# kureta/ddsp-pytorch

Measured on AMD Instinct MI355X. Metric: audio samples/sec/GPU + %HBM-roofline, 16kHz/100-harmonic/batch512, higher is better.
Workload: dtype f32

## Files before the change

ddsp-pytorch_amd/csrc/ddsp_noise_wave.hip:

```cpp
#include <hip/hip_runtime.h>
#include <stdint.h>

#include <atomic>

#include "ddsp_hip.h"
#include "ddsp_internal.h"
#include "ddsp_noise_common.h"

using namespace ddsp_noise;

namespace {

typedef float v4f __attribute__((ext_vector_type(4)));

struct Tile { v4f v[5]; };
struct Lines { v4f v[8]; };
struct Pass { float v[16]; };
struct Spectra { v4f e[2], o[2], h64; float z32; };

constexpr int R = kWaveHop;
constexpr int F = kWaveBands;
constexpr int FG = kWaveGroupFrames;
static_assert(R == 128 && F == 65 && FG == 16 && 2 * (F - 1) == R, "the kernel's register and LDS layouts are written for these");
constexpr int KS = 132;
constexpr int XS = 140;
constexpr int kLdsFloats = FG * KS + FG * XS;

#ifndef DDSP_NOISE_ABL
#define DDSP_NOISE_ABL 0
#endif

#ifdef DDSP_NOISE_STAMPS
#define DDSP_STAMP(i) do { asm volatile("s_waitcnt lgkmcnt(0)" ::: "memory"); const unsigned long long now_ = __builtin_amdgcn_s_memtime(); \
                           stamp_sum[i] += now_ - stamp_last; stamp_last = now_; } while (0)
#else
#define DDSP_STAMP(i) do { } while (0)
#endif

template <bool ACC>
__global__ void __launch_bounds__(64, 2) noise_wave_kernel(NoiseParams p, long ngroups)
{
    extern __shared__ __attribute__((aligned(16))) float smem[];
    float *kern = smem;
    float *xs = smem + FG * KS;
    float *Hs = kern, *ys = xs;
    const int lane = threadIdx.x;
#ifdef DDSP_NOISE_STAMPS
    unsigned long long stamp_sum[8] = {0, 0, 0, 0, 0, 0, 0, 0}, stamp_last = __builtin_amdgcn_s_memtime();
    unsigned long long *stamp_out = reinterpret_cast<unsigned long long *>(const_cast<float *>(p.u)) + 8 * blockIdx.x;
    p.u = nullptr;
#endif

    const int mi0 = lane & 15, mq0 = lane >> 4;
    float *ctab = xs;
    ctab[lane] = cospif((float)lane * (1.0f / 64.0f));
    ctab[lane + 64] = cospif((float)(lane + 64) * (1.0f / 64.0f));
    DDSP_WAVE_ORDER();
    Split Be[2], Bo[2];
#pragma unroll
    for (int t = 0; t < 2; ++t) {
        const int n = 16 * t + mi0;
#pragma unroll
        for (int j = 0; j < 8; ++j) {
            const int k = 8 * mq0 + j;
            split3((k == 0 ? 0.5f : 1.0f) * ctab[(2 * k * n) & 127], Be[t], j);
            split3(ctab[((2 * k + 1) * n) & 127], Bo[t], j);
        }
    }
    float w1[2], w2[2];
#pragma unroll
    for (int t = 0; t < 2; ++t) {
        const int n = 16 * t + mi0;
        w1[t] = __fmaf_rn(0.5f, ctab[n], 0.5f) * (1.0f / 64.0f);
        w2[t] = __fmaf_rn(0.5f, ctab[64 - n], 0.5f) * (1.0f / 64.0f);
    }
    DDSP_WAVE_ORDER();
    const uint64_t base_off = p.offset + (p.offset_dev ? *p.offset_dev : 0ull);

    auto load_tile = [&](long g) {
        const v4f *src = reinterpret_cast<const v4f *>(p.Hm + g * FG * F);
        Tile h;
#pragma unroll
        for (int j = 0; j < 4; ++j) h.v[j] = src[lane + 64 * j];
        h.v[4] = src[256 + (lane & 3)];
        return h;
    };

    auto opaque_lane = [&]() { int ln = lane; asm volatile("" : "+v"(ln)); return ln; };

    auto products = [&](const Tile h) {
        const int ln = opaque_lane(), mi = ln & 15, mq = ln >> 4;
#pragma unroll
        for (int j = 0; j < 4; ++j) *reinterpret_cast<v4f *>(Hs + 4 * (ln + 64 * j)) = h.v[j];
        if (ln < 4) *reinterpret_cast<v4f *>(Hs + 4 * (ln + 256)) = h.v[4];
        DDSP_WAVE_ORDER();
        const float *hrow = Hs + mi * F + 16 * mq;
        float hv[16];
#pragma unroll
        for (int j = 0; j < 16; ++j) hv[j] = hrow[j];
        const float h64 = Hs[mi * F + 64];
        Spectra sp;
#pragma unroll
        for (int r = 0; r < 4; ++r) sp.h64[r] = 0.5f * Hs[(4 * mq + r) * F + 64];
        DDSP_WAVE_ORDER();
        Split Ae, Ao;
#pragma unroll
        for (int j = 0; j < 8; ++j) { split3(hv[2 * j], Ae, j); split3(hv[2 * j + 1], Ao, j); }
        v4f (&accE)[2] = sp.e, (&accO)[2] = sp.o;
        accE[0] = accE[1] = accO[0] = accO[1] = (v4f){0, 0, 0, 0};
        constexpr int PA[6] = {2, 1, 0, 1, 0, 0}, PB[6] = {0, 1, 2, 0, 1, 0};
#pragma unroll
        for (int i = 0; i < (DDSP_NOISE_ABL == 3 ? 1 : 6); ++i) {
            accE[0] = __builtin_amdgcn_mfma_f32_16x16x32_bf16(Ae.p[PA[i]], Be[0].p[PB[i]], accE[0], 0, 0, 0);
            accE[1] = __builtin_amdgcn_mfma_f32_16x16x32_bf16(Ae.p[PA[i]], Be[1].p[PB[i]], accE[1], 0, 0, 0);
            accO[0] = __builtin_amdgcn_mfma_f32_16x16x32_bf16(Ao.p[PA[i]], Bo[0].p[PB[i]], accO[0], 0, 0, 0);
            accO[1] = __builtin_amdgcn_mfma_f32_16x16x32_bf16(Ao.p[PA[i]], Bo[1].p[PB[i]], accO[1], 0, 0, 0);
        }
        float t = (mq == 0 ? 0.5f : 1.0f) * hv[0];
#pragma unroll
        for (int j = 1; j < 8; ++j) t += (j & 1) ? -hv[2 * j] : hv[2 * j];
        t += __shfl_xor(t, 16);
        t += __shfl_xor(t, 32);
        sp.z32 = (t + 0.5f * h64) * (0.5f / 64.0f);
        return sp;
    };

    auto taps = [&](const Spectra sp) {
        const int ln = opaque_lane(), mi = ln & 15, mq = ln >> 4;
        const v4f (&accE)[2] = sp.e, (&accO)[2] = sp.o;
        const float z32 = sp.z32;
#pragma unroll
        for (int t = 0; t < 2; ++t) {
            const int n = 16 * t + mi;
#pragma unroll
            for (int r = 0; r < 4; ++r) {
                float *kr = kern + (4 * mq + r) * KS;
                const float ev = accE[t][r] + ((mi & 1) ? -sp.h64[r] : sp.h64[r]);
                const float v1 = (ev + accO[t][r]) * w1[t];
                const float v2 = (ev - accO[t][r]) * w2[t];
                kr[n] = v1;
                if (n != 0) { kr[128 - n] = v1; kr[64 - n] = v2; }
                kr[64 + n] = v2;
            }
        }
        if (mq == 0) { kern[mi * KS + 32] = z32; kern[mi * KS + 96] = z32; }
        DDSP_WAVE_ORDER();
    };

    auto draw = [&](long frame0) {
        const int ln = opaque_lane();
        for (int e = ln; e < FG * 8; e += 64) xs[(e >> 3) * XS + (e & 7)] = 0.0f;
        if (p.u) {
#pragma unroll
            for (int j = 0; j < 8; ++j) {
                const int qi = ln + 64 * j, fr = qi >> 5, q = qi & 31;
                float4 v = *reinterpret_cast<const float4 *>(p.u + (frame0 + fr) * R + 4 * q);
                v.x = v.x * 2.0f - 1.0f; v.y = v.y * 2.0f - 1.0f; v.z = v.z * 2.0f - 1.0f; v.w = v.w * 2.0f - 1.0f;
                *reinterpret_cast<float4 *>(xs + fr * XS + 8 + 4 * q) = v;
            }
        } else {
            const uint64_t c0 = base_off + (uint64_t)frame0 * 32u + (uint64_t)ln;
#pragma unroll
            for (int j = 0; j < 8; ++j) {
                const int qi = ln + 64 * j, fr = qi >> 5, q = qi & 31;
                const uint64_t ctr = c0 + 64u * j;
                uint32_t rr[4];
                if (DDSP_NOISE_ABL == 2) { rr[0] = (uint32_t)ctr; rr[1] = rr[0] * 3u; rr[2] = rr[0] ^ 77u; rr[3] = rr[0] + 5u; }
                else philox4x32_10((uint32_t)ctr, (uint32_t)(ctr >> 32), (uint32_t)p.seed, (uint32_t)(p.seed >> 32), rr);
                float4 v;
                v.x = philox_to_sample(rr[0]); v.y = philox_to_sample(rr[1]); v.z = philox_to_sample(rr[2]); v.w = philox_to_sample(rr[3]);
                *reinterpret_cast<float4 *>(xs + fr * XS + 8 + 4 * q) = v;
            }
        }
        DDSP_WAVE_ORDER();
    };

    auto conv_pass = [&](int pass) {
        const int ln = opaque_lane();
        const int l5 = ln & 31, seg = l5 >> 2;
        const int cf = ((seg >> 1) << 2) | (l5 & 3);
        const int cs = 2 * (ln >> 5) + ((0x96 >> seg) & 1);
        const float *krow = kern + cf * KS;
        const float *xrow = xs + cf * XS + 8;
        const int cA = pass ? 8 + cs : 15 - cs, cB = 15 - cA;
        const int tsw = cA + 1;
        const float *kq_a = krow, *kq_b = krow - 8 * tsw;
        const float *xq_a = xrow + 8 * cA - 8 - 128, *xq_b = xrow + 8 * cB - 8 + 8 * tsw - 128;
        float acc[8], first[8];
#pragma unroll
        for (int u = 0; u < 8; ++u) { acc[u] = 0.0f; first[u] = 0.0f; }
        float4 cur[6], nxt[6];
        auto fetch = [&](float4 (&d)[6], const float *kq, const float *xq, int t) {
            d[0] = *reinterpret_cast<const float4 *>(kq + 8 * t);
            d[1] = *reinterpret_cast<const float4 *>(kq + 8 * t + 4);
            d[2] = *reinterpret_cast<const float4 *>(xq + 8 * (16 - t));
            d[3] = *reinterpret_cast<const float4 *>(xq + 8 * (16 - t) + 4);
            d[4] = *reinterpret_cast<const float4 *>(xq + 8 * (16 - t) + 8);
            d[5] = *reinterpret_cast<const float4 *>(xq + 8 * (16 - t) + 12);
        };
        fetch(cur, kq_a, xq_a, 0);
#pragma unroll
        for (int t = 0; t < (DDSP_NOISE_ABL == 1 ? 1 : 17); ++t) {
            if (t < 16) {
                if (t + 1 < 9) fetch(nxt, kq_a, xq_a, t + 1);
                else { const bool b = t + 1 >= tsw; fetch(nxt, b ? kq_b : kq_a, b ? xq_b : xq_a, t + 1); }
            }
            if (t >= 9 && t == tsw) {
                asm volatile("" ::: "memory");
#pragma unroll
                for (int u = 0; u < 8; ++u) { first[u] = acc[u]; acc[u] = 0.0f; }
            }
            asm volatile("" ::"v"(cur[2].x));
            const float kv[8] = {cur[0].x, cur[0].y, cur[0].z, cur[0].w, cur[1].x, cur[1].y, cur[1].z, cur[1].w};
            const float xw[16] = {cur[2].x, cur[2].y, cur[2].z, cur[2].w, cur[3].x, cur[3].y, cur[3].z, cur[3].w,
                                  cur[4].x, cur[4].y, cur[4].z, cur[4].w, cur[5].x, cur[5].y, cur[5].z, cur[5].w};
#pragma unroll
            for (int v = 0; v < 8; ++v)
#pragma unroll
                for (int u = 0; u < 8; ++u) acc[u] = __fmaf_rn(kv[v], xw[8 + u - v], acc[u]);
#pragma unroll
            for (int e = 0; e < 6; ++e) cur[e] = nxt[e];
            __builtin_amdgcn_sched_barrier(0);
        }
        Pass out;
#pragma unroll
        for (int u = 0; u < 8; ++u) { out.v[u] = first[u]; out.v[8 + u] = acc[u]; }
        return out;
    };

    auto stage = [&](const Pass r0, const Pass r1) {
        const int ln = opaque_lane();
        const int l5 = ln & 31, seg = l5 >> 2;
        const int cf = ((seg >> 1) << 2) | (l5 & 3);
        const int cs = 2 * (ln >> 5) + ((0x96 >> seg) & 1);
        DDSP_WAVE_ORDER();
#pragma unroll
        for (int pass = 0; pass < 2; ++pass) {
            const float (&r)[16] = pass ? r1.v : r0.v;
            const int cA = pass ? 8 + cs : 15 - cs, cB = 15 - cA;
            float *ya = ys + cf * KS + 8 * cA, *yb = ys + cf * KS + 8 * cB;
            *reinterpret_cast<float4 *>(ya) = make_float4(r[0], r[1], r[2], r[3]);
            *reinterpret_cast<float4 *>(ya + 4) = make_float4(r[4], r[5], r[6], r[7]);
            *reinterpret_cast<float4 *>(yb) = make_float4(r[8], r[9], r[10], r[11]);
            *reinterpret_cast<float4 *>(yb + 4) = make_float4(r[12], r[13], r[14], r[15]);
        }
        DDSP_WAVE_ORDER();
    };

    auto read_y = [&](long frame0) {
        const v4f *src = reinterpret_cast<const v4f *>(p.y) + frame0 * (R / 4);
        Lines yv;
#pragma unroll
        for (int j = 0; j < 8; ++j) yv.v[j] = src[lane + 64 * j];
        return yv;
    };
    auto store_y = [&](long frame0, const Lines yv) {
        const int ln = opaque_lane();
        v4f *dst = reinterpret_cast<v4f *>(p.y) + frame0 * (R / 4);
#pragma unroll
        for (int j = 0; j < 8; ++j) {
            const int i4 = ln + 64 * j;
            v4f o = *reinterpret_cast<const v4f *>(ys + (i4 >> 5) * KS + 4 * (i4 & 31));
            if (ACC && DDSP_NOISE_ABL != 4) o += yv.v[j];
            if (DDSP_NOISE_ABL != 4 || o[0] == 123.0f) dst[i4] = o;
        }
        DDSP_WAVE_ORDER();
    };

    long g = blockIdx.x;
    if (g >= ngroups) return;
    Tile hreg = load_tile(g);
    Lines yv;
#pragma unroll
    for (int j = 0; j < 8; ++j) yv.v[j] = (v4f){0.0f, 0.0f, 0.0f, 0.0f};
    taps(products(hreg));
    draw(g * FG);
    DDSP_STAMP(0);
    for (;;) {
        {
            const unsigned slot = (unsigned)__builtin_amdgcn_s_getreg((4 << 0) | (0 << 6) | (3 << 11));
            const unsigned epoch = (unsigned)(__builtin_amdgcn_s_memrealtime() >> 12);
            if ((slot + epoch) & 1u) __builtin_amdgcn_s_setprio(1); else __builtin_amdgcn_s_setprio(0);
        }
        const long frame0 = g * FG;
        const long gn = g + gridDim.x;
        const Pass r0 = conv_pass(0);
        DDSP_STAMP(1);
        hreg = load_tile(gn < ngroups ? gn : g);
        if (ACC && DDSP_NOISE_ABL != 4) yv = read_y(frame0);
        const Pass r1 = conv_pass(1);
        DDSP_STAMP(2);
        stage(r0, r1);
        DDSP_STAMP(3);
        if (gn >= ngroups) break;
        const Spectra sp = products(hreg);
        DDSP_STAMP(4);
        store_y(frame0, yv);
        DDSP_STAMP(5);
        taps(sp);
        DDSP_STAMP(6);
        draw(gn * FG);
        DDSP_STAMP(7);
        g = gn;
    }
    store_y(g * FG, yv);
#ifdef DDSP_NOISE_STAMPS
    DDSP_STAMP(5);
    if (lane == 0)
        for (int i = 0; i < 8; ++i) stamp_out[i] = stamp_sum[i];
#endif
}

constexpr int kDefaultWavesPerCu = 4;
std::atomic<int> g_residency{0};

}

extern "C" int ddsp_noise_set_residency(int waves_per_cu)
{
    if (waves_per_cu < 0 || waves_per_cu > 8) return DDSP_EINVAL;
    g_residency.store(waves_per_cu, std::memory_order_relaxed);
    return 0;
}
extern "C" int ddsp_noise_get_residency(void)
{
    const int v = g_residency.load(std::memory_order_relaxed);
    return v >= 1 && v <= 8 ? v : kDefaultWavesPerCu;
}

namespace ddsp_noise {

hipError_t launch_noise_wave(const NoiseParams &p, long frames, hipStream_t s)
{
    const long ngroups = frames / FG;
    int cus = 0;
    const hipError_t e = ddsp_device_cus(&cus);
    if (e != hipSuccess) return e;
    constexpr size_t lds = sizeof(float) * kLdsFloats;
    const int asked = g_residency.load(std::memory_order_relaxed);
    const long per_cu = asked >= 1 && asked <= 8 ? asked : kDefaultWavesPerCu;
    long resident = ngroups <= (long)cus * 8 ? (long)cus * 8 : (long)cus * per_cu;
    static const long env_waves = [] { const char *ev = getenv("DDSP_NOISE_WAVES"); return (ev && ddsp_hooks_on()) ? atol(ev) : 0L; }();
    if (env_waves > 0 && env_waves <= 8) resident = (long)cus * env_waves;
    const long grid = ngroups < resident ? ngroups : resident;
    const int slot = ddsp_prof::begin(ddsp_prof::NOISE, s);
    if (p.accumulate) hipLaunchKernelGGL(noise_wave_kernel<true>, dim3((unsigned)grid), dim3(64), lds, s, p, ngroups);
    else hipLaunchKernelGGL(noise_wave_kernel<false>, dim3((unsigned)grid), dim3(64), lds, s, p, ngroups);
    ddsp_prof::end(slot, s);
    return hipGetLastError();
}

}
```

Baseline: 30.85 billion.

## Reuse sliding-window LDS reads in noise conv and simplify draw/store addressing

The convolution inner loop now keeps the previous step's low x-window as the next step's high half, so each step issues four LDS vector loads instead of six. The pass index becomes a compile-time constant, which bounds the window where the kernel-source switch can happen. A reload of the high half is added at that switch. Separately, the tap writes drop the n!=0 branch (the duplicate write at n=0 is harmless), and the zero-fill, draw and store addressing use precomputed per-lane base pointers with fixed strides. The change also adds optional asm phase markers for inspecting the generated code. The main risk is correctness at the switch boundary, plus possible register-pressure changes.

```diff
diff --git a/ddsp-pytorch_amd/csrc/ddsp_noise_wave.hip b/ddsp-pytorch_amd/csrc/ddsp_noise_wave.hip
--- a/ddsp-pytorch_amd/csrc/ddsp_noise_wave.hip
+++ b/ddsp-pytorch_amd/csrc/ddsp_noise_wave.hip
@@ -2,6 +2,7 @@
 #include <stdint.h>
 
 #include <atomic>
+#include <type_traits>
 
 #include "ddsp_hip.h"
 #include "ddsp_internal.h"
@@ -35,6 +36,12 @@
                            stamp_sum[i] += now_ - stamp_last; stamp_last = now_; } while (0)
 #else
 #define DDSP_STAMP(i) do { } while (0)
+#endif
+
+#ifdef DDSP_NOISE_PHASES
+#define DDSP_PHASE(name) asm volatile("; ddsp-phase " name)
+#else
+#define DDSP_PHASE(name) do { } while (0)
 #endif
 
 template <bool ACC>
@@ -138,9 +145,8 @@
                 const float ev = accE[t][r] + ((mi & 1) ? -sp.h64[r] : sp.h64[r]);
                 const float v1 = (ev + accO[t][r]) * w1[t];
                 const float v2 = (ev - accO[t][r]) * w2[t];
-                kr[n] = v1;
-                if (n != 0) { kr[128 - n] = v1; kr[64 - n] = v2; }
-                kr[64 + n] = v2;
+                kr[n] = v1; kr[128 - n] = v1;
+                kr[64 - n] = v2; kr[64 + n] = v2;
             }
         }
         if (mq == 0) { kern[mi * KS + 32] = z32; kern[mi * KS + 96] = z32; }
@@ -149,33 +155,37 @@
 
     auto draw = [&](long frame0) {
         const int ln = opaque_lane();
-        for (int e = ln; e < FG * 8; e += 64) xs[(e >> 3) * XS + (e & 7)] = 0.0f;
+        if (ln < 2 * FG) *reinterpret_cast<float4 *>(xs + (ln >> 1) * XS + 4 * (ln & 1)) = make_float4(0.0f, 0.0f, 0.0f, 0.0f);
+        float *xd = xs + (ln >> 5) * XS + 8 + 4 * (ln & 31);
         if (p.u) {
+            DDSP_PHASE("draw_injected");
+            const float4 *src = reinterpret_cast<const float4 *>(p.u + frame0 * R) + ln;
 #pragma unroll
             for (int j = 0; j < 8; ++j) {
-                const int qi = ln + 64 * j, fr = qi >> 5, q = qi & 31;
-                float4 v = *reinterpret_cast<const float4 *>(p.u + (frame0 + fr) * R + 4 * q);
+                float4 v = src[64 * j];
                 v.x = v.x * 2.0f - 1.0f; v.y = v.y * 2.0f - 1.0f; v.z = v.z * 2.0f - 1.0f; v.w = v.w * 2.0f - 1.0f;
-                *reinterpret_cast<float4 *>(xs + fr * XS + 8 + 4 * q) = v;
+                *reinterpret_cast<float4 *>(xd + 2 * XS * j) = v;
             }
         } else {
+            DDSP_PHASE("draw_philox");
             const uint64_t c0 = base_off + (uint64_t)frame0 * 32u + (uint64_t)ln;
 #pragma unroll
             for (int j = 0; j < 8; ++j) {
-                const int qi = ln + 64 * j, fr = qi >> 5, q = qi & 31;
                 const uint64_t ctr = c0 + 64u * j;
                 uint32_t rr[4];
                 if (DDSP_NOISE_ABL == 2) { rr[0] = (uint32_t)ctr; rr[1] = rr[0] * 3u; rr[2] = rr[0] ^ 77u; rr[3] = rr[0] + 5u; }
                 else philox4x32_10((uint32_t)ctr, (uint32_t)(ctr >> 32), (uint32_t)p.seed, (uint32_t)(p.seed >> 32), rr);
                 float4 v;
                 v.x = philox_to_sample(rr[0]); v.y = philox_to_sample(rr[1]); v.z = philox_to_sample(rr[2]); v.w = philox_to_sample(rr[3]);
-                *reinterpret_cast<float4 *>(xs + fr * XS + 8 + 4 * q) = v;
-            }
-        }
-        DDSP_WAVE_ORDER();
-    };
-
-    auto conv_pass = [&](int pass) {
+                *reinterpret_cast<float4 *>(xd + 2 * XS * j) = v;
+            }
+        }
+        DDSP_WAVE_ORDER();
+    };
+
+    auto conv_pass = [&](auto pass_c) {
+        constexpr int pass = decltype(pass_c)::value;
+        constexpr int T0 = pass ? 9 : 13;
         const int ln = opaque_lane();
         const int l5 = ln & 31, seg = l5 >> 2;
         const int cf = ((seg >> 1) << 2) | (l5 & 3);
@@ -189,37 +199,37 @@
         float acc[8], first[8];
 #pragma unroll
         for (int u = 0; u < 8; ++u) { acc[u] = 0.0f; first[u] = 0.0f; }
-        float4 cur[6], nxt[6];
-        auto fetch = [&](float4 (&d)[6], const float *kq, const float *xq, int t) {
-            d[0] = *reinterpret_cast<const float4 *>(kq + 8 * t);
-            d[1] = *reinterpret_cast<const float4 *>(kq + 8 * t + 4);
-            d[2] = *reinterpret_cast<const float4 *>(xq + 8 * (16 - t));
-            d[3] = *reinterpret_cast<const float4 *>(xq + 8 * (16 - t) + 4);
-            d[4] = *reinterpret_cast<const float4 *>(xq + 8 * (16 - t) + 8);
-            d[5] = *reinterpret_cast<const float4 *>(xq + 8 * (16 - t) + 12);
-        };
-        fetch(cur, kq_a, xq_a, 0);
+        float4 kc[2], lo[2], hi[2], kn[2], lon[2];
+        auto ld4 = [](const float *q) { return *reinterpret_cast<const float4 *>(q); };
+        kc[0] = ld4(kq_a); kc[1] = ld4(kq_a + 4);
+        lo[0] = ld4(xq_a + 128); lo[1] = ld4(xq_a + 132); hi[0] = ld4(xq_a + 136); hi[1] = ld4(xq_a + 140);
 #pragma unroll
         for (int t = 0; t < (DDSP_NOISE_ABL == 1 ? 1 : 17); ++t) {
             if (t < 16) {
-                if (t + 1 < 9) fetch(nxt, kq_a, xq_a, t + 1);
-                else { const bool b = t + 1 >= tsw; fetch(nxt, b ? kq_b : kq_a, b ? xq_b : xq_a, t + 1); }
-            }
-            if (t >= 9 && t == tsw) {
+                const int t1 = t + 1;
+                const float *kq, *xq;
+                if (t1 < T0) { kq = kq_a; xq = xq_a; }
+                else if (t1 >= T0 + 4) { kq = kq_b; xq = xq_b; }
+                else { const bool b = t1 >= tsw; kq = b ? kq_b : kq_a; xq = b ? xq_b : xq_a; }
+                kn[0] = ld4(kq + 8 * t1); kn[1] = ld4(kq + 8 * t1 + 4);
+                lon[0] = ld4(xq + 8 * (16 - t1)); lon[1] = ld4(xq + 8 * (16 - t1) + 4);
+            }
+            if (t >= T0 && t < T0 + 4 && t == tsw) {
                 asm volatile("" ::: "memory");
+                hi[0] = ld4(xq_b + 8 * (16 - t) + 8); hi[1] = ld4(xq_b + 8 * (16 - t) + 12);
 #pragma unroll
                 for (int u = 0; u < 8; ++u) { first[u] = acc[u]; acc[u] = 0.0f; }
             }
-            asm volatile("" ::"v"(cur[2].x));
-            const float kv[8] = {cur[0].x, cur[0].y, cur[0].z, cur[0].w, cur[1].x, cur[1].y, cur[1].z, cur[1].w};
-            const float xw[16] = {cur[2].x, cur[2].y, cur[2].z, cur[2].w, cur[3].x, cur[3].y, cur[3].z, cur[3].w,
-                                  cur[4].x, cur[4].y, cur[4].z, cur[4].w, cur[5].x, cur[5].y, cur[5].z, cur[5].w};
+            asm volatile("" ::"v"(lo[0].x));
+            const float kv[8] = {kc[0].x, kc[0].y, kc[0].z, kc[0].w, kc[1].x, kc[1].y, kc[1].z, kc[1].w};
+            const float xw[16] = {lo[0].x, lo[0].y, lo[0].z, lo[0].w, lo[1].x, lo[1].y, lo[1].z, lo[1].w,
+                                  hi[0].x, hi[0].y, hi[0].z, hi[0].w, hi[1].x, hi[1].y, hi[1].z, hi[1].w};
 #pragma unroll
             for (int v = 0; v < 8; ++v)
 #pragma unroll
                 for (int u = 0; u < 8; ++u) acc[u] = __fmaf_rn(kv[v], xw[8 + u - v], acc[u]);
 #pragma unroll
-            for (int e = 0; e < 6; ++e) cur[e] = nxt[e];
+            for (int e = 0; e < 2; ++e) { kc[e] = kn[e]; hi[e] = lo[e]; lo[e] = lon[e]; }
             __builtin_amdgcn_sched_barrier(0);
         }
         Pass out;
@@ -256,13 +266,13 @@
     };
     auto store_y = [&](long frame0, const Lines yv) {
         const int ln = opaque_lane();
-        v4f *dst = reinterpret_cast<v4f *>(p.y) + frame0 * (R / 4);
+        v4f *dst = reinterpret_cast<v4f *>(p.y) + frame0 * (R / 4) + ln;
+        const float *yrow = ys + (ln >> 5) * KS + 4 * (ln & 31);
 #pragma unroll
         for (int j = 0; j < 8; ++j) {
-            const int i4 = ln + 64 * j;
-            v4f o = *reinterpret_cast<const v4f *>(ys + (i4 >> 5) * KS + 4 * (i4 & 31));
+            v4f o = *reinterpret_cast<const v4f *>(yrow + 2 * KS * j);
             if (ACC && DDSP_NOISE_ABL != 4) o += yv.v[j];
-            if (DDSP_NOISE_ABL != 4 || o[0] == 123.0f) dst[i4] = o;
+            if (DDSP_NOISE_ABL != 4 || o[0] == 123.0f) dst[64 * j] = o;
         }
         DDSP_WAVE_ORDER();
     };
@@ -277,6 +287,7 @@
     draw(g * FG);
     DDSP_STAMP(0);
     for (;;) {
+        DDSP_PHASE("turn");
         {
             const unsigned slot = (unsigned)__builtin_amdgcn_s_getreg((4 << 0) | (0 << 6) | (3 << 11));
             const unsigned epoch = (unsigned)(__builtin_amdgcn_s_memrealtime() >> 12);
@@ -284,24 +295,33 @@
         }
         const long frame0 = g * FG;
         const long gn = g + gridDim.x;
-        const Pass r0 = conv_pass(0);
+        DDSP_PHASE("conv_pass0");
+        const Pass r0 = conv_pass(std::integral_constant<int, 0>{});
         DDSP_STAMP(1);
+        DDSP_PHASE("loads");
         hreg = load_tile(gn < ngroups ? gn : g);
         if (ACC && DDSP_NOISE_ABL != 4) yv = read_y(frame0);
-        const Pass r1 = conv_pass(1);
+        DDSP_PHASE("conv_pass1");
+        const Pass r1 = conv_pass(std::integral_constant<int, 1>{});
         DDSP_STAMP(2);
+        DDSP_PHASE("stage");
         stage(r0, r1);
         DDSP_STAMP(3);
         if (gn >= ngroups) break;
+        DDSP_PHASE("products");
         const Spectra sp = products(hreg);
         DDSP_STAMP(4);
+        DDSP_PHASE("store_y");
         store_y(frame0, yv);
         DDSP_STAMP(5);
+        DDSP_PHASE("taps");
         taps(sp);
         DDSP_STAMP(6);
+        DDSP_PHASE("draw");
         draw(gn * FG);
         DDSP_STAMP(7);
         g = gn;
+        DDSP_PHASE("next");
     }
     store_y(g * FG, yv);
 #ifdef DDSP_NOISE_STAMPS
```

After: 31.12 billion (median of 6 runs). No clear change (+0.9%).
